# minh86/ModelCrowdNav

Measured on NVIDIA B200. Metric: env-steps/s (ORCA step + SARL lookahead), higher is better.
Workload: dtype f16

## Files before the change

modelcrowdnav_b200/csrc/lookahead_tc.cu:

```cuda
#include "env_math.cuh"
#include "umma.cuh"

#include <cuda_fp16.h>
#include <math.h>
#include <stdlib.h>
#include <string.h>

#include <vector>

int cn_lookahead_prepare(cn_policy *p, cn_env *env, cudaStream_t s);
int cn_lookahead_argmax(cn_policy *p, cn_env *env, double epsilon, cudaStream_t s, bool pdl);

namespace {

using namespace umma;

constexpr int K_X = 32;
constexpr int N_H1 = 160;
constexpr int N_M1 = 112;
constexpr int N_F = 64;
constexpr int K_A1 = 224;
constexpr int K_J = 80;
constexpr int ROWS = 128;

// ... 286 lines not shown
    const double dt = p.time_step;
    for (int idx = threadIdx.x; idx < kOmItems * H; idx += blockDim.x) {
        const int it = idx / H, j = idx - it * H;
        const long long item = item0 + it;
        int cell = -1;
        double vxr = 0.0, vyr = 0.0;
        if (item < n_items) {
            const int e = (int)(item / H), i = (int)(item - (long long)e * H);
            auto get = [&](int k, int f) -> double {
                const double vx = query_env ? human_v[(size_t)(0 * H + k) * ed.E + e] : st[st_idx(ed, F_VX, k + 1, e)];
                const double vy = query_env ? human_v[(size_t)(1 * H + k) * ed.E + e] : st[st_idx(ed, F_VY, k + 1, e)];
                if (f == 0) return st[st_idx(ed, F_PX, k + 1, e)] + vx * dt;
                if (f == 1) return st[st_idx(ed, F_PY, k + 1, e)] + vy * dt;
                return f == 2 ? vx : vy;
            };
            if (j != i) cell = occupancy_map_pair(d, i, j, get, vxr, vyr);
        }
        cell_of[it][j] = cell;
        vrot_of[it][j][0] = vxr; vrot_of[it][j][1] = vyr;
    }
    __syncthreads();
    for (int idx = threadIdx.x; idx < kOmItems * cells; idx += blockDim.x) {
        const int it = idx / cells, c = idx - it * cells;
        double cnt = 0.0, sx = 0.0, sy = 0.0;
        for (int j = 0; j < H; ++j)
            if (cell_of[it][j] == c) { cnt += 1.0; sx += vrot_of[it][j][0]; sy += vrot_of[it][j][1]; }
        occupancy_map_store(d.om_ch, c, cnt, sx, sy, om[it]);
    }
    __syncthreads();
    const int n = threadIdx.x;
    float acc[kOmItems];
#pragma unroll
    for (int it = 0; it < kOmItems; ++it) acc[it] = 0.0f;
    if (n < m10.out)
        for (int k = 0; k < d.om_dim; ++k) {
            const float w = m10.wt[(size_t)(13 + k) * m10.ld + n];
#pragma unroll
            for (int it = 0; it < kOmItems; ++it) acc[it] = fmaf(om[it][k], w, acc[it]);
        }
#pragma unroll
    for (int it = 0; it < kOmItems; ++it)
        if (item0 + it < n_items) P[(size_t)(item0 + it) * N_H1 + n] = acc[it];
}

int cn_tc_init(cn_policy *p)
{
    const SarlDims &d = p->d;
    if (d.net == CN_NET_CADRL) {
        if (!(d.in == 13 && d.m3[0] == 150 && d.m3[1] == 100 && d.m3[2] == 100 && d.m3[3] == 1)) {
            cn_set_error("CN_PREC_F16_TC is specialised for the default [cadrl] mlp_dims (150, 100, 100, 1); use CN_PREC_F32 "
                         "for other shapes");
            return CN_EUNSUPPORTED;
        }
    } else if (d.net == CN_NET_LSTM_RL) {
        if (!(d.in == 13 && d.self_dim == 6 && d.lstm_h == L_HIDDEN && d.lm1[0] == 0 && d.om_dim == 0 && d.m3[0] == 150 &&
              d.m3[1] == 100 && d.m3[2] == 100 && d.m3[3] == 1)) {
            cn_set_error("CN_PREC_F16_TC runs LSTM-RL's default shape only (no interaction module, no occupancy maps, "
                         "global_state_dim 50, mlp2_dims 150,100,100,1); use CN_PREC_F32 for other shapes");
            return CN_EUNSUPPORTED;
        }
    } else {
        const bool ok = d.net == CN_NET_SARL && d.in == 13 + d.om_dim && d.self_dim == 6 && d.m1[0] == 150 && d.m1[1] == 100 &&
                        d.m2[0] == 100 && d.m2[1] == 50 && d.at[0] == 100 && d.at[1] == 100 && d.at[2] == 1 &&
                        d.m3[0] == 150 && d.m3[1] == 100 && d.m3[2] == 100 && d.m3[3] == 1;
        if (!ok) {
            cn_set_error("CN_PREC_F16_TC is specialised for the default [sarl] dims (150,100 / 100,50 / 100,100,1 / "
                         "150,100,100,1) and the default [cadrl] mlp_dims; use CN_PREC_F32 for other shapes / networks");
            return CN_EUNSUPPORTED;
        }
    }
    TcState *t = new TcState();
    memset(t, 0, sizeof(*t));
    p->tc = t;
    cudaDeviceProp prop;
    CN_CUDA_CHECK(cudaGetDeviceProperties(&prop, p->device));
    t->num_sms = prop.multiProcessorCount;
    for (const auto &by_om : kRowsKernels)
        for (const auto &by_ht : by_om)
            for (RowsKernel k : by_ht) CN_CUDA_CHECK(cudaFuncSetAttribute(k, cudaFuncAttributeMaxDynamicSharedMemorySize, (int)Q_SMEM));
    CN_CUDA_CHECK(cudaFuncSetAttribute(tc_mlp3_pair_kernel<0>, cudaFuncAttributeMaxDynamicSharedMemorySize, (int)M_SMEM));
    CN_CUDA_CHECK(cudaFuncSetAttribute(tc_mlp3_pair_kernel<1>, cudaFuncAttributeMaxDynamicSharedMemorySize, (int)M_SMEM));
    CN_CUDA_CHECK(cudaFuncSetAttribute(tc_lstm_pair_kernel, cudaFuncAttributeMaxDynamicSharedMemorySize, (int)L_SMEM));
    if (cudaMalloc((void **)&t->img_pair, 2 * IMG_H_BYTES) != cudaSuccess ||
        cudaMalloc((void **)&t->img_lstm, 2 * IMG_HL_BYTES) != cudaSuccess ||
        cudaMalloc((void **)&t->img_pair_b, 2 * IMG_HM_BYTES) != cudaSuccess) {
        cn_set_error("cudaMalloc failed for the tensor-core weight images");
        return CN_ENOMEM;
    }
    return CN_OK;
}

void cn_tc_destroy(cn_policy *p)
{
    TcState *t = (TcState *)p->tc;
    if (!t) return;
    if (t->img_pair) cudaFree(t->img_pair);
    if (t->img_pair_b) cudaFree(t->img_pair_b);
    if (t->J) cudaFree(t->J);
    if (t->X) cudaFree(t->X);
    if (t->rew) cudaFree(t->rew);
    if (t->rowv) cudaFree(t->rowv);
    if (t->omP) cudaFree(t->omP);
    if (t->img_lstm) cudaFree(t->img_lstm);
    if (t->XL) cudaFree(t->XL);
    if (t->ord) cudaFree(t->ord);
    if (t->dbg) cudaFree(t->dbg);
    if (t->kev[0]) for (int i = 0; i < 5; ++i) cudaEventDestroy(t->kev[i]);
    delete t;
    p->tc = nullptr;
}

int cn_tc_load_weights(cn_policy *p, const float *flat, cudaStream_t s)
{
    TcState *t = (TcState *)p->tc;
    const SarlDims &d = p->d;
    std::vector<HostLinear> L;
    const float *lstm = nullptr, *src = flat;
    for (const LayerSpec &l : cn_layers(d, p->w)) {
        if (l.dst_hh) lstm = src;
        else L.push_back({src, src + (size_t)l.in * l.out, l.in, l.out});
        src += cn_layer_floats(l);
    }
    const std::vector<uint8_t> hb = mlp3_image(&L[L.size() - 4], d.net == CN_NET_CADRL, t->tail_b);
    std::vector<uint8_t> hp, hl;
    CN_CUDA_CHECK(cudaMemcpyAsync(t->img_pair_b, hb.data(), hb.size(), cudaMemcpyHostToDevice, s));
    if (d.net == CN_NET_SARL) {
        hp = rows_image(L.data(), !d.no_gs, t->tail_a);
        CN_CUDA_CHECK(cudaMemcpyAsync(t->img_pair, hp.data(), hp.size(), cudaMemcpyHostToDevice, s));
    } else if (d.net == CN_NET_LSTM_RL) {
        hl = lstm_image(lstm);
        CN_CUDA_CHECK(cudaMemcpyAsync(t->img_lstm, hl.data(), hl.size(), cudaMemcpyHostToDevice, s));
    }
    CN_CUDA_CHECK(cudaStreamSynchronize(s));
    return CN_OK;
}

int cn_lookahead_tc(cn_policy *p, cn_env *env, int query_env, double epsilon, cudaStream_t s, cudaStream_t tail)
{
    TcState *t = (TcState *)p->tc;
    const EnvDims ed = env->p.d;
    if (ed.H > CN_MAX_HUMANS) { cn_set_error("human_num too large"); return CN_EUNSUPPORTED; }
    int rc = cn_lookahead_prepare(p, env, s);
    if (rc) return rc;
    const bool pipelined = tail && tail != s;
    const int net = p->d.net, A = p->d.A;
    const bool om = p->d.om_dim > 0;
    const size_t NG = (size_t)ed.E * A;
    int G = ROWS / ed.H;
    if (G > 64) G = 64;
    const PairGrid ga = pair_grid(t->num_sms, (int)((NG + G - 1) / G));
    const PairGrid gb = pair_grid(t->num_sms, (int)((NG + ROWS - 1) / ROWS));
    if ((rc = cn_grow(t->J, t->cap_jtiles, (NG + ROWS - 1) / ROWS + 4 * (size_t)(t->num_sms / 2), J_TILE_BYTES, true, s))) return rc;
    if ((rc = cn_grow(t->rew, t->cap_rew, NG, sizeof(double)))) return rc;
    if ((rc = cn_grow(t->X, t->cap_xtiles, ga.tiles, X_TILE_BYTES))) return rc;
    const double gamma_bar = pow(p->cfg.gamma, env->p.time_step * p->cfg.v_pref);
    TailW twa, twb;
    memcpy(twa.w, t->tail_a, sizeof(twa.w));
    memcpy(twb.w, t->tail_b, sizeof(twb.w));
    const int ht = (ed.H == 5 && G == ROWS / 5) ? 5 : ((ed.H == 10 && G == ROWS / 10) ? 10 : 0);
    auto feat = ht == 5 ? tc_features_kernel<5> : (ht == 10 ? tc_features_kernel<10> : tc_features_kernel<0>);

    if ((rc = stamp(t, 0, "features", s))) return rc;
    feat<<<(unsigned)ga.tiles, ROWS, 0, s>>>(env->p, env->state, env->time, env->human_v, p->action_dev, A, query_env, (int)NG, G,
                                             env->theta, t->X, t->J, t->rew);
    CN_LAUNCH_CHECK();
    if ((rc = stamp(t, 1, "rows", s))) return rc;
    if (net == CN_NET_LSTM_RL) {
        if ((rc = cn_grow(t->XL, t->cap_xl, gb.tiles * ed.H, X_TILE_BYTES))) return rc;
        if ((rc = cn_grow(t->ord, t->cap_ord, (size_t)ed.E * ed.H, sizeof(int32_t)))) return rc;
        lstm_order_kernel<<<(ed.E + 127) / 128, 128, 0, s>>>(env->p, env->state, query_env, t->ord);
        CN_LAUNCH_CHECK();
        tc_features_lstm_kernel<<<(unsigned)(gb.tiles * ed.H), ROWS, 0, s>>>(env->p, env->state, env->time, env->human_v, p->action_dev,
                                                                           A, query_env, (int)NG, env->theta, t->ord, t->XL);
        CN_LAUNCH_CHECK();
        tc_lstm_pair_kernel<<<2 * gb.clusters, kThreadsL, L_SMEM, s>>>(t->img_lstm, t->XL, t->J, ed.H, gb.rounds);
        CN_LAUNCH_CHECK();
    } else if (net == CN_NET_CADRL) {
        if ((rc = cn_grow(t->rowv, t->cap_rowv, ga.tiles * ROWS, sizeof(float)))) return rc;
        if ((rc = cn_launch(tc_mlp3_pair_kernel<1>, 2 * ga.clusters, kThreadsM3, M_SMEM, s, false, env->p, env->state, t->img_pair_b,
                            t->X, t->rew, A, (int)NG, p->cfg.gamma, gamma_bar, p->cfg.v_pref, p->values, ga.rounds, twb, t->rowv)))
            return rc;
    } else {
        if (om) {
            const size_t items = (size_t)ed.E * ed.H;
            if ((rc = cn_grow(t->omP, t->cap_om, items, sizeof(float) * N_H1))) return rc;
            tc_om_bias_kernel<<<(unsigned)((items + kOmItems - 1) / kOmItems), N_H1, 0, s>>>(env->p, p->d, p->w.m1[0], env->state,
                                                                                          env->human_v, query_env, t->omP);
            CN_LAUNCH_CHECK();
        }
        const RowsKernel rows = kRowsKernels[p->d.no_gs ? 1 : 0][om ? 1 : 0][ht == 5 ? 1 : (ht == 10 ? 2 : 0)];
        if ((rc = cn_launch(rows, 2 * ga.clusters, kThreadsPair, Q_SMEM, s, !om && !pipelined, env->p, t->img_pair, t->X, t->J, (int)NG,
                            G, ga.rounds, twa, t->dbg, t->omP, A)))
            return rc;
    }
    if (pipelined) {
        CN_CUDA_CHECK(cudaEventRecord(env->ev_rows, s));
        CN_CUDA_CHECK(cudaStreamWaitEvent(tail, env->ev_rows, 0));
        s = tail;
    }
    if ((rc = stamp(t, 2, "mlp3", s))) return rc;
    if (net == CN_NET_CADRL) {
        cadrl_min_kernel<<<(unsigned)((NG + 255) / 256), 256, 0, s>>>(env->p, env->state, t->rowv, t->rew, A, (int)NG, G, ed.H,
                                                                      p->cfg.gamma, gamma_bar, p->cfg.v_pref, p->values);
        CN_LAUNCH_CHECK();
    } else if ((rc = cn_launch(tc_mlp3_pair_kernel<0>, 2 * gb.clusters, kThreadsM3, M_SMEM, s, net != CN_NET_LSTM_RL, env->p,
                                 env->state, t->img_pair_b, t->J, t->rew, A, (int)NG, p->cfg.gamma, gamma_bar, p->cfg.v_pref,
                                 p->values, gb.rounds, twb, nullptr))) {
        return rc;
    }
    if ((rc = stamp(t, 3, "argmax", s))) return rc;
    if ((rc = cn_lookahead_argmax(p, env, epsilon, s, !pipelined))) return rc;
    return stamp(t, 4, nullptr, s);
}

static int selftest_impl(int32_t N, int32_t K, const float *a_host, const float *b_host, float *d_host, int device, int mode)
{
    const int bmn = mode == 1;
    if (N < 16 || N > 256 || N % 16 || K < 16 || K % 16 || K > 256 || (bmn && K > ROWS)) {
        cn_set_error("N in [16,256] step 16, K in [16,256] step 16 (K <= 128 for the MN-major variant)");
        return CN_EINVAL;
    }
    int n = 0;
    if (cudaGetDeviceCount(&n) != cudaSuccess || n == 0) { cudaGetLastError(); cn_set_error("no CUDA device available; no CPU fallback"); return CN_ECUDA; }
    CN_CUDA_CHECK(cudaSetDevice(device));
    std::vector<uint8_t> ai(bytes_of(ROWS, K), 0), bi(bmn ? bytes_of(ROWS, N) : bytes_of(N, K), 0);
    for (int r = 0; r < ROWS; ++r) for (int k = 0; k < K; ++k) put(ai, 0, ROWS, r, k, a_host[(size_t)r * K + k]);
    for (int r = 0; r < N; ++r)
        for (int k = 0; k < K; ++k) {
            if (bmn) put(bi, 0, ROWS, k, r, b_host[(size_t)r * K + k]);
            else put(bi, 0, N, r, k, b_host[(size_t)r * K + k]);
        }
    uint8_t *da = nullptr, *db = nullptr;
    float *dd = nullptr;
    CN_CUDA_CHECK(cudaMalloc((void **)&da, ai.size()));
    CN_CUDA_CHECK(cudaMalloc((void **)&db, bi.size()));
    CN_CUDA_CHECK(cudaMalloc((void **)&dd, sizeof(float) * ROWS * N));
    CN_CUDA_CHECK(cudaMemcpy(da, ai.data(), ai.size(), cudaMemcpyHostToDevice));
    CN_CUDA_CHECK(cudaMemcpy(db, bi.data(), bi.size(), cudaMemcpyHostToDevice));
    const size_t smem = ai.size() + bi.size() + 64;
    CN_CUDA_CHECK(cudaFuncSetAttribute(umma_selftest_kernel, cudaFuncAttributeMaxDynamicSharedMemorySize, (int)smem));
    umma_selftest_kernel<<<1, 128, smem>>>(da, db, dd, N, K, mode);
    CN_LAUNCH_CHECK();
    CN_CUDA_CHECK(cudaDeviceSynchronize());
    CN_CUDA_CHECK(cudaMemcpy(d_host, dd, sizeof(float) * ROWS * N, cudaMemcpyDeviceToHost));
    cudaFree(da); cudaFree(db); cudaFree(dd);
    return CN_OK;
}

extern "C" int cn_selftest_umma(int32_t N, int32_t K, const float *a_host, const float *b_host, float *d_host, int device)
{
    return selftest_impl(N, K, a_host, b_host, d_host, device, 0);
}

extern "C" int cn_selftest_umma_bmn(int32_t N, int32_t K, const float *a_host, const float *b_host, float *d_host, int device)
{
    return selftest_impl(N, K, a_host, b_host, d_host, device, 1);
}

extern "C" int cn_selftest_umma_ts(int32_t N, int32_t K, const float *a_host, const float *b_host, float *d_host, int device)
{
    return selftest_impl(N, K, a_host, b_host, d_host, device, 2);
}

extern "C" int cn_selftest_umma_pair(int32_t N, int32_t K, const float *a_host, const float *b_host, float *d_host,
                                     int32_t reps, long long *cycles_host, int device)
{
    if (N < 32 || N > 256 || N % 16 || K < 16 || K % 16 || K > 256 || reps < 1) {
        cn_set_error("N in [32,256] step 16, K in [16,256] step 16, reps >= 1");
        return CN_EINVAL;
    }
    int n = 0;
    if (cudaGetDeviceCount(&n) != cudaSuccess || n == 0) { cudaGetLastError(); cn_set_error("no CUDA device available; no CPU fallback"); return CN_ECUDA; }
    CN_CUDA_CHECK(cudaSetDevice(device));
    const size_t a_bytes = bytes_of(ROWS, K), b_bytes = bytes_of(N / 2, K);
    std::vector<uint8_t> ai(2 * a_bytes, 0), bi(2 * b_bytes, 0);
    for (int r = 0; r < 2 * ROWS; ++r)
        for (int k = 0; k < K; ++k) put(ai, (uint32_t)((r / ROWS) * a_bytes), ROWS, r % ROWS, k, a_host[(size_t)r * K + k]);
    for (int r = 0; r < N; ++r)
        for (int k = 0; k < K; ++k) put(bi, (uint32_t)((r / (N / 2)) * b_bytes), N / 2, r % (N / 2), k, b_host[(size_t)r * K + k]);
    uint8_t *da = nullptr, *db = nullptr;
    float *dd = nullptr;
    long long *dc = nullptr;
    CN_CUDA_CHECK(cudaMalloc((void **)&da, ai.size()));
    CN_CUDA_CHECK(cudaMalloc((void **)&db, bi.size()));
    CN_CUDA_CHECK(cudaMalloc((void **)&dd, sizeof(float) * 2 * ROWS * N));
    CN_CUDA_CHECK(cudaMalloc((void **)&dc, sizeof(long long)));
    CN_CUDA_CHECK(cudaMemcpy(da, ai.data(), ai.size(), cudaMemcpyHostToDevice));
    CN_CUDA_CHECK(cudaMemcpy(db, bi.data(), bi.size(), cudaMemcpyHostToDevice));
    const size_t smem = a_bytes + b_bytes + 64;
    CN_CUDA_CHECK(cudaFuncSetAttribute(umma_pair_selftest_kernel, cudaFuncAttributeMaxDynamicSharedMemorySize, (int)smem));
    umma_pair_selftest_kernel<<<2, 160, smem>>>(da, db, dd, N, K, reps, dc);
    CN_LAUNCH_CHECK();
    CN_CUDA_CHECK(cudaDeviceSynchronize());
    CN_CUDA_CHECK(cudaMemcpy(d_host, dd, sizeof(float) * 2 * ROWS * N, cudaMemcpyDeviceToHost));
    if (cycles_host) CN_CUDA_CHECK(cudaMemcpy(cycles_host, dc, sizeof(long long), cudaMemcpyDeviceToHost));
    cudaFree(da); cudaFree(db); cudaFree(dd); cudaFree(dc);
    return CN_OK;
}

extern "C" int cn_debug_tc_timing(cn_policy *p, long long *out16)
{
    if (!p || !p->tc) { cn_set_error("policy has no tensor-core state"); return CN_EINVAL; }
    TcState *t = (TcState *)p->tc;
    CN_CUDA_CHECK(cudaSetDevice(p->device));
    if (!t->dbg) {
        CN_CUDA_CHECK(cudaMalloc((void **)&t->dbg, 256 * sizeof(long long)));
        CN_CUDA_CHECK(cudaMemset(t->dbg, 0, 256 * sizeof(long long)));
    }
    CN_CUDA_CHECK(cudaDeviceSynchronize());
    CN_CUDA_CHECK(cudaMemcpy(out16, t->dbg, 256 * sizeof(long long), cudaMemcpyDeviceToHost));
    return CN_OK;
}

extern "C" int cn_debug_kernel_ms(cn_policy *p, int on, float *out4)
{
    if (!p || !p->tc) { cn_set_error("policy has no tensor-core state"); return CN_EINVAL; }
    TcState *t = (TcState *)p->tc;
// ... 11 lines not shown
```

modelcrowdnav_b200/csrc/tc_rows_pair.cuh:

```cuda

constexpr int kThreadsPair = 608;
constexpr int N_S2 = 2 * N_M1;
constexpr int PAIR_CTX_COLS = 256;
constexpr int T_H1B = 80;
constexpr int T_D1 = 120;
constexpr int T_A2 = N_M1 / 2;
constexpr int T_F = T_A2 + N_M1;

constexpr uint32_t H_W1 = 0;
constexpr uint32_t H_W2 = H_W1 + bytes_of(N_H1 / 2, K_X);
constexpr uint32_t H_W3A = H_W2 + bytes_of(N_M1 / 2, N_H1);
constexpr uint32_t H_WB = H_W3A + bytes_of(N_M1, N_M1);
constexpr uint32_t H_W4 = H_WB + bytes_of(N_M1 / 2, N_M1);
constexpr uint32_t H_WA2 = H_W4 + bytes_of(N_F / 2, N_M1);
constexpr uint32_t H_TAIL = H_WA2 + bytes_of(N_M1 / 2, N_M1);
constexpr uint32_t IMG_H_BYTES = H_TAIL + TAIL_BYTES;

constexpr uint32_t Q_R1_BYTES = bytes_of(ROWS, N_H1);
constexpr uint32_t Q_R2_BYTES = bytes_of(ROWS, N_M1);
constexpr uint32_t Q_X_OFF = bytes_of(ROWS, N_M1);
constexpr uint32_t Q_CTX_BYTES = Q_R1_BYTES + Q_R2_BYTES;
constexpr uint32_t Q_CTX0 = (IMG_H_BYTES + 127) & ~127u;
constexpr uint32_t Q_MISC = Q_CTX0 + 2 * Q_CTX_BYTES;
constexpr uint32_t Q_SMEM = Q_MISC + 2048 + 2048 + 96 + 16;
static_assert(Q_X_OFF + bytes_of(ROWS, K_X) <= Q_R1_BYTES, "next-tile X must fit behind the 112-column tiles");
static_assert(Q_SMEM <= 232448, "tc_rows_pair_kernel exceeds 227 KB of shared memory");

struct RowInPP {
    double rpx, rpy, rgx, rgy, rr, rvp, hpx, hpy, hvx, hvy, cvx, cvy, hr, ax, ay, t;
    float ntheta;
    int valid;
};

__device__ __forceinline__ void pp_load_inputs(RowInPP &in, const EnvDims &ed, const double *__restrict__ st,
                                               const double *__restrict__ time, const double *__restrict__ human_v,
                                               const double *__restrict__ actions, int A, int query_env, int NG, int G,
                                               int tile, int gl, int h, int kinematics, const double *__restrict__ theta)
{
    const int H = ed.H;
    const int g = tile * G + gl;
    in.valid = (gl < G && g < NG) ? 1 : 0;
    if (!in.valid) return;
    const int e = A == 81 ? g / 81 : g / A, a = g - e * A;
    const size_t fs = (size_t)ed.A1 * ed.E;
    const double *__restrict__ pr = st + e, *__restrict__ ph = pr + (size_t)(h + 1) * ed.E;
    in.rpx = pr[F_PX * fs]; in.rpy = pr[F_PY * fs];
    in.rgx = pr[F_GX * fs]; in.rgy = pr[F_GY * fs];
    in.rr = pr[F_R * fs];   in.rvp = pr[F_VPREF * fs];
    in.hpx = ph[F_PX * fs]; in.hpy = ph[F_PY * fs];
    in.hr = ph[F_R * fs];
    in.cvx = ph[F_VX * fs]; in.cvy = ph[F_VY * fs];
    if (query_env) {
        in.hvx = human_v[(size_t)(0 * H + h) * ed.E + e]; in.hvy = human_v[(size_t)(1 * H + h) * ed.E + e];
        in.t = time[e];
    } else {
        in.hvx = in.cvx; in.hvy = in.cvy; in.t = 0.0;
    }
    const double a0 = actions[2 * a], a1 = actions[2 * a + 1];
    const double th = kinematics != CN_KIN_HOLONOMIC ? theta[e] : 0.0;
    cn_effective_velocity(kinematics, th, a0, a1, in.ax, in.ay);
    in.ntheta = kinematics != CN_KIN_HOLONOMIC ? (float)(th + a1) : 0.0f;
}

__device__ __forceinline__ double pp_clearance(const RowInPP &in, double dt, int query_env)
{
    if (!in.valid) return INFINITY;
    if (query_env) {
        const double px = in.hpx - in.rpx, py = in.hpy - in.rpy;
        const double vx = in.cvx - in.ax, vy = in.cvy - in.ay;
        const double ex = px + vx * dt, ey = py + vy * dt;
        return cn_point_to_segment_dist0(px, py, ex, ey) - in.hr - in.rr;
    }
    const double npx = in.rpx + in.ax * dt, npy = in.rpy + in.ay * dt;
    const double nhx = in.hpx + in.cvx * dt, nhy = in.hpy + in.cvy * dt;
    const double dx = npx - nhx, dy = npy - nhy;
    const float fx = (float)dx, fy = (float)dy, fr = (float)in.rr + (float)in.hr + 0.25f;
    if (fx * fx + fy * fy > fr * fr) return 1.0e30;
    return norm2d(dx, dy) - in.rr - in.hr;
}

__device__ __forceinline__ void rotate_dir(const float *s, float *o, int kinematics)
{
    const float dx = s[5] - s[0], dy = s[6] - s[1];
    const float d = sqrtf(dx * dx + dy * dy);
    float c = 1.0f, sn = 0.0f;
    if (d > 0.0f) { const float inv = 1.0f / d; c = dx * inv; sn = dy * inv; }
    o[0] = d;
    o[1] = s[7];
    o[2] = kinematics == CN_KIN_UNICYCLE ? s[8] - atan2f(dy, dx) : 0.0f;
    o[3] = s[4];
    o[4] = s[2] * c + s[3] * sn;
    o[5] = s[3] * c - s[2] * sn;
    o[6] = (s[9] - s[0]) * c + (s[10] - s[1]) * sn;
    o[7] = (s[10] - s[1]) * c - (s[9] - s[0]) * sn;
    o[8] = s[11] * c + s[12] * sn;
    o[9] = s[12] * c - s[11] * sn;
    o[10] = s[13];
    const float ax = s[0] - s[9], ay = s[1] - s[10];
    o[11] = sqrtf(ax * ax + ay * ay);
    o[12] = s[4] + s[13];
}

__device__ __forceinline__ void pair_features(const RowInPP &in, double dt, int kinematics, uint4 &c0, uint4 &c1, uint4 &c2,
                                              uint4 &c3)
{
    c0 = make_uint4(0, 0, 0, 0); c1 = c0; c2 = c0; c3 = c0;
    if (!in.valid) return;
    float s[14], o[13];
    s[0] = (float)(in.rpx + in.ax * dt); s[1] = (float)(in.rpy + in.ay * dt);
    s[2] = (float)in.ax; s[3] = (float)in.ay; s[4] = (float)in.rr;
    s[5] = (float)in.rgx; s[6] = (float)in.rgy; s[7] = (float)in.rvp; s[8] = in.ntheta;
    s[9] = (float)(in.hpx + in.hvx * dt); s[10] = (float)(in.hpy + in.hvy * dt);
    s[11] = (float)in.hvx; s[12] = (float)in.hvy; s[13] = (float)in.hr;
    rotate_dir(s, o, kinematics);
    float hi[13], lo[13];
#pragma unroll
    for (int k = 0; k < 13; ++k) split_hl(o[k], hi[k], lo[k]);
    c0 = make_uint4(h2(hi[0], hi[1]), h2(hi[2], hi[3]), h2(hi[4], hi[5]), h2(hi[6], hi[7]));
    c1 = make_uint4(h2(hi[8], hi[9]), h2(hi[10], hi[11]), h2(hi[12], 1.0f), h2(1.0f, 0.0f));
    c2 = make_uint4(h2(lo[0], lo[1]), h2(lo[2], lo[3]), h2(lo[4], lo[5]), h2(lo[6], lo[7]));
    c3 = make_uint4(h2(lo[8], lo[9]), h2(lo[10], lo[11]), h2(lo[12], 0.0f), 0u);
}

__device__ __forceinline__ double pair_reward(const EnvParams &p, const RowInPP &in, const double *__restrict__ D, int H,
                                              int query_env)
{
    const double dt = p.time_step;
    double dmin = INFINITY;
    bool collision = false;
    for (int k = 0; k < H; ++k) {
        const double c = D[k];
        if (c < 0) collision = true;
        else if (c < dmin) dmin = c;
    }
    const double npx = in.rpx + in.ax * dt, npy = in.rpy + in.ay * dt;
    const bool reaching_goal = norm2d(npx - in.rgx, npy - in.rgy) < in.rr;
    if (query_env) {
        if (in.t >= p.time_limit - 1) return 0;
        if (collision) return p.collision_penalty;
        if (reaching_goal) return p.success_reward;
        if (dmin < p.discomfort_dist) return (dmin - p.discomfort_dist) * p.discomfort_penalty_factor * dt;
        return 0;
    }
    if (collision) return -0.25;
    if (reaching_goal) return 1;
    if (dmin < 0.2) return (dmin - 0.2) * 0.5 * dt;
    return 0;
}


struct TailW { float w[104]; };

constexpr uint32_t X_TILE_BYTES = bytes_of(ROWS, K_X);

template <int HT>
__global__ void __launch_bounds__(ROWS, 9)
tc_features_kernel(EnvParams p, const double *__restrict__ st, const double *__restrict__ time,
                   const double *__restrict__ human_v, const double *__restrict__ actions, int A, int query_env, int NG,
                   int G_rt, const double *__restrict__ theta, uint8_t *__restrict__ X, uint8_t *__restrict__ J,
                   double *__restrict__ rew)
{
    __shared__ double D[ROWS];
    pdl_launch_dependents();
    const EnvDims ed = p.d;
    const int H = HT ? HT : ed.H;
    const int G = HT ? ROWS / HT : G_rt;
    const int tile = blockIdx.x, r = threadIdx.x;
    const int gl = r / H, h = r - gl * H;
    const double dt = p.time_step;
    RowInPP in;
    pp_load_inputs(in, ed, st, time, human_v, actions, A, query_env, NG, G, tile, gl, h, p.kinematics, theta);
    D[r] = pp_clearance(in, dt, query_env);
    uint4 c0, c1, c2, c3;
    pair_features(in, dt, p.kinematics, c0, c1, c2, c3);
    uint8_t *xt = X + (size_t)tile * X_TILE_BYTES;
    *reinterpret_cast<uint4 *>(xt + chunk_off(ROWS, r, 0)) = c0;
    *reinterpret_cast<uint4 *>(xt + chunk_off(ROWS, r, 1)) = c1;
    *reinterpret_cast<uint4 *>(xt + chunk_off(ROWS, r, 2)) = c2;
    *reinterpret_cast<uint4 *>(xt + chunk_off(ROWS, r, 3)) = c3;
    const bool lead = in.valid && h == 0;
    const int g = tile * G + gl;
    if (lead) {
        uint8_t *jt = J + (size_t)(g >> 7) * J_TILE_BYTES;
        const int rb = g & 127;
        *reinterpret_cast<uint4 *>(jt + chunk_off(ROWS, rb, 7)) = make_uint4(c0.x, c0.y, c0.z, h2(1.0f, 1.0f));
        *reinterpret_cast<uint4 *>(jt + chunk_off(ROWS, rb, 8)) = make_uint4(c2.x, c2.y, c2.z, 0u);
        *reinterpret_cast<uint4 *>(jt + chunk_off(ROWS, rb, 9)) = make_uint4(0, 0, 0, 0);
    }
    __syncthreads();
    if (r < G && tile * G + r < NG) {
        RowInPP in0;
        pp_load_inputs(in0, ed, st, time, human_v, actions, A, query_env, NG, G, tile, r, 0, p.kinematics, theta);
        rew[tile * G + r] = pair_reward(p, in0, D + r * H, H, query_env);
    }
}

__device__ __forceinline__ void sum_f16x8_rows(const uint8_t *base, int n, uint32_t stride, float (&acc)[8])
{
    for (int i0 = 0; i0 < n; i0 += 4) {
        uint4 u[4];
#pragma unroll
        for (int j = 0; j < 4; ++j)
            u[j] = (i0 + j < n) ? *reinterpret_cast<const uint4 *>(base + (size_t)(i0 + j) * stride) : make_uint4(0, 0, 0, 0);
#pragma unroll
        for (int j = 0; j < 4; ++j) {
            const __half2 *hv = reinterpret_cast<const __half2 *>(&u[j]);
#pragma unroll
            for (int k = 0; k < 4; ++k) { const float2 f = __half22float2(hv[k]); acc[2 * k] += f.x; acc[2 * k + 1] += f.y; }
        }
    }
}

__device__ __forceinline__ void ctx_barrier(int ctx)
{
    if (ctx == 0) asm volatile("bar.sync 1, 256;" ::: "memory");
    else asm volatile("bar.sync 2, 256;" ::: "memory");
}

template <int HT, bool OM, bool GS>
__global__ void __cluster_dims__(2, 1, 1) __maxnreg__(88)
tc_rows_pair_kernel(EnvParams p,
                    const uint8_t *__restrict__ wimg, const uint8_t *__restrict__ X, uint8_t *__restrict__ J, int NG, int G_rt,
                    int rounds, const TailW tw, long long *__restrict__ dbg, const float *__restrict__ omP, int A)
{
#define QPROBE(slot, i) do { if (dbg && blockIdx.x < 2 && probe_round) dbg[(blockIdx.x * 4 + (slot)) * 32 + (i)] = clock64(); } while (0)
    extern __shared__ __align__(128) uint8_t smem[];
    const EnvDims ed = p.d;
    const int H = HT ? HT : ed.H;
    const int G = HT ? ROWS / HT : G_rt;
    const int tid = threadIdx.x, warp = tid >> 5, lane = tid & 31;
    const bool is_issuer_warp = warp == 16, is_producer_warp = warp > 16;
    const int q = warp & 3, ctx = (warp >> 2) & 1, hf = (warp >> 3) & 1;
    const uint32_t rank = cluster_ctarank();
    const int cluster_id = blockIdx.x >> 1, nclusters = gridDim.x >> 1;
    const int row = q * 32 + lane;
    const int t256 = hf * 128 + row;
    const int my_gl = row / H, my_h = row - my_gl * H;
    const int rows = G * H;
    uint8_t *R1 = smem + Q_CTX0 + (uint32_t)ctx * Q_CTX_BYTES, *R2 = R1 + Q_R1_BYTES;
    float *S0 = reinterpret_cast<float *>(smem + Q_MISC) + ctx * 256, *S1 = S0 + 128;
    const uint32_t bar0 = smem_u32(smem + Q_MISC + 4096);
    const uint32_t req0 = bar0, req1 = bar0 + 8, done0 = bar0 + 16, done1 = bar0 + 24, reqm0 = bar0 + 32, reqm1 = bar0 + 40;
    const uint32_t xfull0 = bar0 + 48, xfull1 = bar0 + 56;
    const uint32_t xland0 = bar0 + 80, xland1 = bar0 + 88;
    const uint32_t xfree0 = bar0 + 64, xfree1 = bar0 + 72;
    uint32_t *tmem_slot = reinterpret_cast<uint32_t *>(smem + Q_MISC + 4096 + 96);

    copy_image_to_smem(smem, wimg + (size_t)rank * IMG_H_BYTES, IMG_H_BYTES);
    for (uint32_t i = tid * 16; i < 2 * Q_CTX_BYTES; i += kThreadsPair * 16)
        *reinterpret_cast<uint4 *>(smem + Q_CTX0 + i) = make_uint4(0, 0, 0, 0);
    if (tid == 0) {
        mbar_init(req0, 16); mbar_init(req1, 16); mbar_init(done0, 1); mbar_init(done1, 1);
        mbar_init(reqm0, 16); mbar_init(reqm1, 16);
        mbar_init(xfull0, 2); mbar_init(xfull1, 2); mbar_init(xfree0, 1); mbar_init(xfree1, 1);
        mbar_init(xland0, 1); mbar_init(xland1, 1);
        fence_mbar_init();
    }
    if (warp == 0) tmem_alloc_2(smem_u32(tmem_slot), 512);
    fence_async_smem();
    fence_before_sync();
    __syncthreads();
    cluster_sync_all();
    fence_after_sync();
    const uint32_t tmem = *tmem_slot;
    pdl_launch_dependents();
    pdl_wait();

    if (is_issuer_warp) {
        if (rank == 0 && lane == 0) {
            const uint32_t sW1 = smem_u32(smem + H_W1), sW2 = smem_u32(smem + H_W2), sW3A = smem_u32(smem + H_W3A);
            const uint32_t sWB = smem_u32(smem + H_WB), sW4 = smem_u32(smem + H_W4), sWA2 = smem_u32(smem + H_WA2);
            constexpr int NS = GS ? 5 : 4;
            const int total = NS * rounds;
            int stage0 = 0, stage1 = 0;
            uint32_t ph0 = 0, ph1 = 0, phm0 = 0, phm1 = 0, phx0 = 0, phx1 = 0;
            uint32_t idle_polls = 0;
            while (stage0 < total || stage1 < total) {
#pragma unroll
                for (int c = 0; c < 2; ++c) {
                    int &stage = c ? stage1 : stage0;
                    if (stage >= total) continue;
                    const int s = stage % NS;
                    uint32_t &ph = (GS && s == 3) ? (c ? phm1 : phm0) : (c ? ph1 : ph0);
                    if (!mbar_test_wait_cluster((GS && s == 3) ? (c ? reqm1 : reqm0) : (c ? req1 : req0), ph)) continue;
                    if (s == 0) {
                        uint32_t &phx = c ? phx1 : phx0;
                        if (!mbar_test_wait_cluster(c ? xfull1 : xfull0, phx)) continue;
                        phx ^= 1;
                    }
                    ph ^= 1;
                    const bool probe_round = stage / NS == 3;
                    QPROBE(2 + c, 2 * s);
                    fence_after_sync();
                    const uint32_t tm = tmem + (uint32_t)c * PAIR_CTX_COLS;
                    const uint32_t sR1 = smem_u32(smem + Q_CTX0 + (uint32_t)c * Q_CTX_BYTES), sR2 = sR1 + Q_R1_BYTES;
                    const uint32_t done = c ? done1 : done0;
#ifdef CN_ABLATE_MMA
                    if (!GS || s != 2) commit_2(done, 3);
                    if (1) {
                    } else if (s == 0) {
#else
                    if (s == 0) {
#endif
                        mma_layer_2(tm, sR1 + Q_X_OFF, ROWS, sW1, K_X, N_H1, false);
                        commit_2(done, 3);
                    } else if (s == 1) {
                        mma_steps_2_ts(tm + T_D1, tm, sW2, 0, N_H1 / 32, N_M1, false);
                        mma_steps_2_ts(tm + T_D1, tm + T_H1B, sW2, N_H1 / 32, N_H1 / 16, N_M1, true);
                        commit_2(done, 3);
                    } else if (s == 2) {
                        mma_layer_2(tm, sR2, ROWS, sW3A, N_M1, N_S2, false);
                        if constexpr (!GS) commit_2(done, 3);
                    } else if (GS && s == 3) {
                        mma_layer_2(tm, sR1, ROWS, sWB, N_M1, N_M1, true);
                        commit_2(done, 3);
                    } else {
                        mma_steps_2_ts(tm + T_A2, tm, sWA2, 0, N_M1 / 16, N_M1, false);
                        mma_layer_2(tm + T_F, sR1, ROWS, sW4, N_M1, N_F, false);
                        commit_2(done, 3);
                    }
                    QPROBE(2 + c, 2 * s + 1);
                    ++stage;
                    idle_polls = 0;
                }
                if (++idle_polls > (1u << 28)) __trap();
            }
        }
    } else if (is_producer_warp) {
        if (lane == 0) {
            const int c = warp - 17;
            const uint32_t xl = c ? xland1 : xland0, xfree = c ? xfree1 : xfree0;
            const uint32_t xfull_leader = mapa(c ? xfull1 : xfull0, 0);
            const uint32_t dst = smem_u32(smem + Q_CTX0 + (uint32_t)c * Q_CTX_BYTES + Q_X_OFF);
            const int tile_stride = 4 * nclusters;
            int tile = (cluster_id * 2 + (int)rank) * 2 + c;
            uint32_t phf = 0, phl = 0;
            for (int rnd = 0; rnd < rounds; ++rnd, tile += tile_stride) {
                if (rnd > 0) { mbar_wait_guarded(xfree, phf); phf ^= 1; }
                bulk_load(dst, X + (size_t)tile * X_TILE_BYTES, X_TILE_BYTES, xl);
                mbar_wait_guarded(xl, phl); phl ^= 1;
                mbar_arrive_cluster(xfull_leader);
            }
        }
    } else {
        const uint32_t done = ctx ? done1 : done0;
        const uint32_t req_leader = mapa(ctx ? req1 : req0, 0), reqm_leader = mapa(ctx ? reqm1 : reqm0, 0);
        const uint32_t tl = tmem + ((uint32_t)(q * 32) << 16) + (uint32_t)ctx * PAIR_CTX_COLS;
        uint32_t ph = 0;
        const float invH = 1.0f / (float)H;
        const int tile_stride = 4 * nclusters;
        int tile = (cluster_id * 2 + (int)rank) * 2 + ctx;
        constexpr int kMeanIters = HT ? 2 : 4;
        int mean_off[kMeanIters];
#pragma unroll
        for (int i = 0; i < kMeanIters; ++i) {
            const int it = t256 + i * 256;
            const int c = it / G, gl = it - c * G;
            mean_off[i] = (it < G * (N_M1 / 8)) ? (int)chunk_off(ROWS, gl * H, c) : -1;
        }
        constexpr int kSumIters = HT ? 1 : 2;
        auto pow2_floor = [](int x) { int p = 1; while (2 * p <= x && p < 16) p *= 2; return p; };
        const int mean_split = HT ? 1 : pow2_floor(256 / (G * (N_M1 / 8)));
        const int sum_split = HT ? 1 : pow2_floor(256 / (G * 7));
        uint8_t *mean_scratch = R1 + Q_X_OFF + X_TILE_BYTES;
        static_assert(Q_X_OFF + X_TILE_BYTES + 2 * ROWS * 4 <= Q_R1_BYTES, "softmax scratch must fit behind the X slot");
#define PAIR_SIGNAL_TO(bar) do { fence_async_smem(); fence_before_sync(); __syncwarp(); if (lane == 0) mbar_arrive_cluster(bar); } while (0)
#define PAIR_SIGNAL() PAIR_SIGNAL_TO(req_leader)
#define PAIR_WAIT() do { mbar_wait_guarded(done, ph); ph ^= 1; fence_after_sync(); } while (0)
        auto om_prefetch = [&](int tl_idx) {
            const long long g2 = (long long)tl_idx * G + my_gl;
            if (row < rows && g2 < NG) {
                const float *b = omP + ((size_t)(g2 / A) * H + my_h) * N_H1 + hf * 80;
                asm volatile("prefetch.global.L1 [%0];" :: "l"(b));
                asm volatile("prefetch.global.L1 [%0];" :: "l"(b + 32));
                asm volatile("prefetch.global.L1 [%0];" :: "l"(b + 64));
            }
        };
        if constexpr (OM) om_prefetch(tile);
        PAIR_SIGNAL();
        for (int rnd = 0; rnd < rounds; ++rnd, tile += tile_stride) {
            const bool has_next = rnd + 1 < rounds;
            const bool probe_round = (t256 == 0) && rnd == 3;
            const long long g = (long long)tile * G + my_gl;
            const bool row_valid = (row < rows) && (g < NG);
            QPROBE(ctx, 0);
            PAIR_WAIT(); QPROBE(ctx, 1);
            if (warp == 4 * ctx && lane == 0) mbar_arrive(ctx ? xfree1 : xfree0);
            if constexpr (OM) {
                const float *bias = row_valid ? omP + ((size_t)(g / A) * H + my_h) * N_H1 + hf * 80 : nullptr;
                compact_to_tmem_bias(tl, hf * 80, 80, hf * T_H1B, bias);
            } else
#ifndef CN_ABLATE_EPI
            compact_to_tmem<true, true>(tl, hf * 80, 80, hf * T_H1B, 1.0f);
#endif
            PAIR_SIGNAL(); QPROBE(ctx, 2);
            if constexpr (OM) { if (has_next) om_prefetch(tile + tile_stride); }
            PAIR_WAIT(); QPROBE(ctx, 3);
#ifndef CN_ABLATE_EPI
            if (hf == 0) epilogue_to_smem<true>(tl, T_D1, 64, R2, row, 0);
            else epilogue_to_smem<true>(tl, T_D1 + 64, 48, R2, row, 8);
#endif
            PAIR_SIGNAL(); QPROBE(ctx, 4);
            if constexpr (GS) {
                QPROBE(ctx, 12);
                ctx_barrier(ctx);
                QPROBE(ctx, 13);
#ifdef CN_ABLATE_EPI
                if (0) {
#else
                if (!HT && mean_split >= 2) {
#endif
                    const int P = mean_split, nitems = G * (N_M1 / 8);
                    const int it = t256 / P, seg = t256 & (P - 1);
                    const bool on = it < nitems;
                    const int c = on ? it / G : 0, gl = on ? it - c * G : 0;
                    const int n = on ? (H - seg + P - 1) / P : 0;
                    float acc[8] = {0, 0, 0, 0, 0, 0, 0, 0};
                    sum_f16x8_rows(R2 + chunk_off(ROWS, gl * H + seg, c), n, 16u * P, acc);
                    for (int off = 1; off < P; off <<= 1)
#pragma unroll
                        for (int k = 0; k < 8; ++k) acc[k] += __shfl_xor_sync(0xffffffffu, acc[k], off);
                    const uint4 o = make_uint4(h2(acc[0] * invH, acc[1] * invH), h2(acc[2] * invH, acc[3] * invH),
                                               h2(acc[4] * invH, acc[5] * invH), h2(acc[6] * invH, acc[7] * invH));
                    for (int h = seg; h < H && on; h += P)
                        *reinterpret_cast<uint4 *>(R1 + chunk_off(ROWS, gl * H + h, c)) = o;
                } else
#pragma unroll
                for (int i = 0; i < kMeanIters; ++i) {
#ifdef CN_ABLATE_EPI
                    break;
#endif
                    if (mean_off[i] < 0) continue;
                    const uint8_t *src = R2 + mean_off[i];
                    uint4 v[HT ? HT : 1];
                    __half2 acc[4];
                    if (HT) {
#pragma unroll
                        for (int h = 0; h < HT; ++h) v[h] = *reinterpret_cast<const uint4 *>(src + h * 16);
                        const __half2 *h0 = reinterpret_cast<const __half2 *>(&v[0]);
                        acc[0] = h0[0]; acc[1] = h0[1]; acc[2] = h0[2]; acc[3] = h0[3];
#pragma unroll
                        for (int h = 1; h < HT; ++h) {
                            const __half2 *hv = reinterpret_cast<const __half2 *>(&v[h]);
#pragma unroll
                            for (int k = 0; k < 4; ++k) acc[k] = __hadd2(acc[k], hv[k]);
                        }
                    } else {
                        v[0] = *reinterpret_cast<const uint4 *>(src);
                        const __half2 *h0 = reinterpret_cast<const __half2 *>(&v[0]);
                        acc[0] = h0[0]; acc[1] = h0[1]; acc[2] = h0[2]; acc[3] = h0[3];
                        for (int h = 1; h < H; ++h) {
                            const uint4 u = *reinterpret_cast<const uint4 *>(src + h * 16);
                            const __half2 *hv = reinterpret_cast<const __half2 *>(&u);
#pragma unroll
                            for (int k = 0; k < 4; ++k) acc[k] = __hadd2(acc[k], hv[k]);
                        }
                    }
                    uint4 o;
                    {
                        const float2 f0 = __half22float2(acc[0]), f1 = __half22float2(acc[1]);
                        const float2 f2 = __half22float2(acc[2]), f3 = __half22float2(acc[3]);
                        o.x = h2(f0.x * invH, f0.y * invH); o.y = h2(f1.x * invH, f1.y * invH);
                        o.z = h2(f2.x * invH, f2.y * invH); o.w = h2(f3.x * invH, f3.y * invH);
                    }
                    uint8_t *dst = R1 + mean_off[i];
                    if (HT) {
#pragma unroll
                        for (int h = 0; h < HT; ++h) *reinterpret_cast<uint4 *>(dst + h * 16) = o;
                    } else {
                        for (int h = 0; h < H; ++h) *reinterpret_cast<uint4 *>(dst + h * 16) = o;
                    }
                }
                QPROBE(ctx, 14);
                PAIR_SIGNAL_TO(reqm_leader); QPROBE(ctx, 5);
                if (dbg && blockIdx.x < 2 && rnd == 3 && ctx == 0 && lane == 0) dbg[192 + blockIdx.x * 8 + hf * 4 + q] = clock64();
            }
            QPROBE(ctx, 6);
            PAIR_WAIT(); QPROBE(ctx, 7);
#ifndef CN_ABLATE_EPI
            if (hf == 0) compact_to_tmem<true, true>(tl, 0, N_M1, 0, 1.0f);
            else epilogue_to_smem<true>(tl, N_M1, N_M1, R1, row, 0);
#endif
            PAIR_SIGNAL(); QPROBE(ctx, 8);
            PAIR_WAIT(); QPROBE(ctx, 9);
#ifdef CN_ABLATE_EPI
            if (has_next) PAIR_SIGNAL();
            ctx_barrier(ctx);
            QPROBE(ctx, 11);
            continue;
#endif
            {
                float part = 0.0f;
                if (hf == 0) {
                    uint32_t v[32];
                    ld32(tl + T_A2, v);
// ... 208 lines not shown
```

Before: 12.11 million.

## Store only human half of pair features and rebuild X tiles in smem

For non-CADRL nets, the features kernel now writes only the human-specific 16-column half of each X tile, halving X global writes and the producer's bulk loads. The producer warp then reassembles the full 32-column tile in shared memory by gathering each group's self features from the J tiles and interleaving them with the loaded human chunks before signalling the cluster leader. This trades global traffic for extra per-lane gathers from J, smem shuffling and an async-proxy fence on the producer's critical path, and it depends on the exact packing of the c0..c3 words.

```diff
diff --git a/modelcrowdnav_b200/csrc/lookahead_tc.cu b/modelcrowdnav_b200/csrc/lookahead_tc.cu
--- a/modelcrowdnav_b200/csrc/lookahead_tc.cu
+++ b/modelcrowdnav_b200/csrc/lookahead_tc.cu
@@ -462,7 +462,8 @@
     const PairGrid gb = pair_grid(t->num_sms, (int)((NG + ROWS - 1) / ROWS));
     if ((rc = cn_grow(t->J, t->cap_jtiles, (NG + ROWS - 1) / ROWS + 4 * (size_t)(t->num_sms / 2), J_TILE_BYTES, true, s))) return rc;
     if ((rc = cn_grow(t->rew, t->cap_rew, NG, sizeof(double)))) return rc;
-    if ((rc = cn_grow(t->X, t->cap_xtiles, ga.tiles, X_TILE_BYTES))) return rc;
+    const int full_x = net == CN_NET_CADRL;
+    if ((rc = cn_grow(t->X, t->cap_xtiles, ga.tiles, full_x ? X_TILE_BYTES : X_HUMAN_TILE_BYTES))) return rc;
     const double gamma_bar = pow(p->cfg.gamma, env->p.time_step * p->cfg.v_pref);
     TailW twa, twb;
     memcpy(twa.w, t->tail_a, sizeof(twa.w));
@@ -472,7 +473,7 @@
 
     if ((rc = stamp(t, 0, "features", s))) return rc;
     feat<<<(unsigned)ga.tiles, ROWS, 0, s>>>(env->p, env->state, env->time, env->human_v, p->action_dev, A, query_env, (int)NG, G,
-                                             env->theta, t->X, t->J, t->rew);
+                                             env->theta, full_x, t->X, t->J, t->rew);
     CN_LAUNCH_CHECK();
     if ((rc = stamp(t, 1, "rows", s))) return rc;
     if (net == CN_NET_LSTM_RL) {
diff --git a/modelcrowdnav_b200/csrc/tc_rows_pair.cuh b/modelcrowdnav_b200/csrc/tc_rows_pair.cuh
--- a/modelcrowdnav_b200/csrc/tc_rows_pair.cuh
+++ b/modelcrowdnav_b200/csrc/tc_rows_pair.cuh
@@ -152,12 +152,13 @@
 struct TailW { float w[104]; };
 
 constexpr uint32_t X_TILE_BYTES = bytes_of(ROWS, K_X);
+constexpr uint32_t X_HUMAN_TILE_BYTES = bytes_of(ROWS, K_X / 2);
 
 template <int HT>
 __global__ void __launch_bounds__(ROWS, 9)
 tc_features_kernel(EnvParams p, const double *__restrict__ st, const double *__restrict__ time,
                    const double *__restrict__ human_v, const double *__restrict__ actions, int A, int query_env, int NG,
-                   int G_rt, const double *__restrict__ theta, uint8_t *__restrict__ X, uint8_t *__restrict__ J,
+                   int G_rt, const double *__restrict__ theta, int full_x, uint8_t *__restrict__ X, uint8_t *__restrict__ J,
                    double *__restrict__ rew)
 {
     __shared__ double D[ROWS];
@@ -173,11 +174,17 @@
     D[r] = pp_clearance(in, dt, query_env);
     uint4 c0, c1, c2, c3;
     pair_features(in, dt, p.kinematics, c0, c1, c2, c3);
-    uint8_t *xt = X + (size_t)tile * X_TILE_BYTES;
-    *reinterpret_cast<uint4 *>(xt + chunk_off(ROWS, r, 0)) = c0;
-    *reinterpret_cast<uint4 *>(xt + chunk_off(ROWS, r, 1)) = c1;
-    *reinterpret_cast<uint4 *>(xt + chunk_off(ROWS, r, 2)) = c2;
-    *reinterpret_cast<uint4 *>(xt + chunk_off(ROWS, r, 3)) = c3;
+    if (full_x) {
+        uint8_t *xt = X + (size_t)tile * X_TILE_BYTES;
+        *reinterpret_cast<uint4 *>(xt + chunk_off(ROWS, r, 0)) = c0;
+        *reinterpret_cast<uint4 *>(xt + chunk_off(ROWS, r, 1)) = c1;
+        *reinterpret_cast<uint4 *>(xt + chunk_off(ROWS, r, 2)) = c2;
+        *reinterpret_cast<uint4 *>(xt + chunk_off(ROWS, r, 3)) = c3;
+    } else {
+        uint8_t *xt = X + (size_t)tile * X_HUMAN_TILE_BYTES;
+        *reinterpret_cast<uint4 *>(xt + chunk_off(ROWS, r, 0)) = make_uint4(c0.w, c1.x, c1.y, c1.z);
+        *reinterpret_cast<uint4 *>(xt + chunk_off(ROWS, r, 1)) = make_uint4(c2.w, c3.x, c3.y, c3.z);
+    }
     const bool lead = in.valid && h == 0;
     const int g = tile * G + gl;
     if (lead) {
@@ -327,20 +334,41 @@
             }
         }
     } else if (is_producer_warp) {
-        if (lane == 0) {
-            const int c = warp - 17;
-            const uint32_t xl = c ? xland1 : xland0, xfree = c ? xfree1 : xfree0;
-            const uint32_t xfull_leader = mapa(c ? xfull1 : xfull0, 0);
-            const uint32_t dst = smem_u32(smem + Q_CTX0 + (uint32_t)c * Q_CTX_BYTES + Q_X_OFF);
-            const int tile_stride = 4 * nclusters;
-            int tile = (cluster_id * 2 + (int)rank) * 2 + c;
-            uint32_t phf = 0, phl = 0;
-            for (int rnd = 0; rnd < rounds; ++rnd, tile += tile_stride) {
-                if (rnd > 0) { mbar_wait_guarded(xfree, phf); phf ^= 1; }
-                bulk_load(dst, X + (size_t)tile * X_TILE_BYTES, X_TILE_BYTES, xl);
-                mbar_wait_guarded(xl, phl); phl ^= 1;
-                mbar_arrive_cluster(xfull_leader);
-            }
+        const int c = warp - 17;
+        const uint32_t xl = c ? xland1 : xland0, xfree = c ? xfree1 : xfree0;
+        const uint32_t xfull_leader = mapa(c ? xfull1 : xfull0, 0);
+        uint8_t *slot = smem + Q_CTX0 + (uint32_t)c * Q_CTX_BYTES + Q_X_OFF;
+        const int tile_stride = 4 * nclusters;
+        int tile = (cluster_id * 2 + (int)rank) * 2 + c;
+        uint32_t phf = 0, phl = 0;
+        for (int rnd = 0; rnd < rounds; ++rnd, tile += tile_stride) {
+            if (rnd > 0) { mbar_wait_guarded(xfree, phf); phf ^= 1; }
+            if (lane == 0) bulk_load(smem_u32(slot + 2 * ROWS * 16), X + (size_t)tile * X_HUMAN_TILE_BYTES, X_HUMAN_TILE_BYTES, xl);
+            mbar_wait_guarded(xl, phl); phl ^= 1;
+            uint4 self_hi[4], self_lo[4];
+#pragma unroll
+            for (int i = 0; i < 4; ++i) {
+                const int r = lane + 32 * i, g = tile * G + r / H;
+                self_hi[i] = make_uint4(0, 0, 0, 0); self_lo[i] = self_hi[i];
+                if (r < rows && g < NG) {
+                    const uint8_t *jr = J + (size_t)(g >> 7) * J_TILE_BYTES + chunk_off(ROWS, g & 127, 7);
+                    self_hi[i] = *reinterpret_cast<const uint4 *>(jr);
+                    self_lo[i] = *reinterpret_cast<const uint4 *>(jr + ROWS * 16);
+                }
+            }
+#pragma unroll
+            for (int i = 0; i < 4; ++i) {
+                uint4 *x0 = reinterpret_cast<uint4 *>(slot + chunk_off(ROWS, lane + 32 * i, 0));
+                uint4 *x1 = x0 + ROWS, *x2 = x1 + ROWS, *x3 = x2 + ROWS;
+                const uint4 hh = *x2, hl = *x3;
+                *x0 = make_uint4(self_hi[i].x, self_hi[i].y, self_hi[i].z, hh.x);
+                *x1 = make_uint4(hh.y, hh.z, hh.w, self_hi[i].w & 0xffffu);
+                *x2 = make_uint4(self_lo[i].x, self_lo[i].y, self_lo[i].z, hl.x);
+                *x3 = make_uint4(hl.y, hl.z, hl.w, 0u);
+            }
+            fence_async_smem();
+            __syncwarp();
+            if (lane == 0) mbar_arrive_cluster(xfull_leader);
         }
     } else {
         const uint32_t done = ctx ? done1 : done0;
```

New measurement: 12.20 million (median of 6 runs). No clear change (+0.8%).
